# luisdamiano/sparseRGPs

Hardware: AMD Instinct MI355X
Metric: sparse-GP objective+gradient evals/sec at n=1e6, m=1024, d=8 (higher is better)
Workload: dtype f64; 1 GPU; C3: Titsias VI ELBO + gradient, n=1000000, m=1024, d=8, ard, P=10, knots fixed; n=1000000, m=1024, d=8, kernel=ard, parallelism=single

## Files before the change

include/sgp_diag.h:

```cpp
#ifndef SGP_DIAG_H
#define SGP_DIAG_H

#include <stdint.h>

#ifdef __cplusplus
extern "C" {
#endif

int sgp_diag_gj_pair(int device, int64_t m, const double* A, const double* B, double beta,
                     int per_step, double* invA, double* invS, double* logdet);

int sgp_diag_store_bw(int device, int64_t bytes, int reps, int pattern, double* gbs);

#ifdef __cplusplus
}
#endif
#endif
```

sparsergps_amd/_build.py:

```python
from __future__ import annotations

import os
import shutil
import subprocess

HERE = os.path.dirname(os.path.abspath(__file__))
ROOT = os.path.dirname(HERE)
CSRC = os.path.join(HERE, "csrc")
LIBDIR = os.path.join(HERE, "lib")
LIB = os.path.join(LIBDIR, "libsgp.so")
VARIANT_ROOT = os.path.join(ROOT, "tools", "ab")
SOURCES = ["capi.hip", "k_cov.hip", "k_mfma.hip", "k_dense.hip", "k_lap.hip", "multi.hip"]
HEADERS = ["sgp_internal.h", "sgp_probe.h", "sgp_multi.h", "sgp_pool.h",
           os.path.join("..", "..", "include", "sgp.h"),
           os.path.join("..", "..", "include", "sgp_diag.h")]
ARCH = "gfx950"


class HipccMissing(RuntimeError):
    """No hipcc on this machine (the only case in which an existing library may be reused)."""


def hipcc():
    for cand in (shutil.which("hipcc"), "/opt/rocm/bin/hipcc"):
        if cand and os.path.exists(cand):
            return cand
    raise HipccMissing("hipcc not found: cannot build libsgp.so")

# ... 114 lines not shown
        raise RuntimeError("SGP_HIPCC_DEFS is not honoured by the product build; "
                           "use sparsergps_amd._build.build_variant() for A/B libraries")
    return _build_into(LIBDIR, LIB, (), force, verbose)


def build_variant(name: str, defs=(), force: bool = False, verbose: bool = False,
                  rev: str | None = None) -> str:
    if not name or "/" in name or name.startswith("."):
        raise ValueError(f"bad variant name {name!r}")
    defs = ["-DSGP_PROBE_BUILD", *defs]
    outdir = os.path.join(VARIANT_ROOT, name)
    csrc = CSRC
    if rev is not None:
        src_root = os.path.join(outdir, "src")
        os.makedirs(src_root, exist_ok=True)
        for path in ["sparsergps_amd/csrc/" + f for f in SOURCES + HEADERS[:4]] + ["include/sgp.h", "include/sgp_diag.h"]:
            res = subprocess.run(["git", "-C", ROOT, "show", f"{rev}:{path}"],
                                 stdout=subprocess.PIPE, stderr=subprocess.PIPE)
            if res.returncode != 0:
                continue
            out = res.stdout
            dst = os.path.join(src_root, path)
            os.makedirs(os.path.dirname(dst), exist_ok=True)
            old = open(dst, "rb").read() if os.path.exists(dst) else None
            if old != out:
                with open(dst, "wb") as f:
                    f.write(out)
        csrc = os.path.join(src_root, "sparsergps_amd", "csrc")
    return _build_into(outdir, os.path.join(outdir, "libsgp.so"), defs, force, verbose, csrc)


# ... 9 lines not shown
```

sparsergps_amd/_lib.py:

```python
from __future__ import annotations

import ctypes as C
import os
import threading

from ._build import LIB, VARIANT_ROOT, HipccMissing, build

_lock = threading.Lock()
_lib = None

c_double_p = C.POINTER(C.c_double)
c_int_p = C.POINTER(C.c_int)

SGP_OK, SGP_EINVAL, SGP_ENOTPD, SGP_EHIP, SGP_ENOMEM = 0, 1, 2, 3, 4
KERNELS = {"sqexp": 0, "ard": 1, "exp": 2}
SGP_FLAG_R_DET = 1
SGP_FLAG_OBJ_ONLY = 2
SGP_PRED_VI, SGP_PRED_LAPLACE, SGP_PRED_FULL = 0, 1, 2
SGP_EXPO_ROWS = 0.0
FAMILIES = {"poisson": 0, "bernoulli": 1}

PROTOTYPES = {
    "sgp_last_error": (C.c_char_p, []),
    "sgp_abi_version": (C.c_int, []),
# ... 30 lines not shown
                                C.c_double, C.c_void_p]),
    "sgp_vi_phase2": (C.c_int, [C.c_void_p, C.c_void_p, C.c_int64, C.c_uint, C.c_void_p]),
    "sgp_vi_finish": (C.c_int, [C.c_void_p, C.c_void_p, c_double_p, c_double_p]),
    "sgp_fitc_red1_count": (C.c_int64, [C.c_int64]),
    "sgp_fitc_red2_count": (C.c_int64, [C.c_int, C.c_int, C.c_int64]),
    "sgp_fitc_phase1": (C.c_int, [C.c_void_p, C.c_int, c_double_p, c_double_p, C.c_int64, C.c_int64,
                                  C.c_double, C.c_void_p]),
    "sgp_fitc_phase2": (C.c_int, [C.c_void_p, C.c_void_p, C.c_int64, C.c_uint, C.c_void_p]),
    "sgp_fitc_finish": (C.c_int, [C.c_void_p, C.c_void_p, c_double_p, c_double_p]),
    "sgp_lap_set_f": (C.c_int, [C.c_void_p, c_double_p, C.c_double]),
    "sgp_lap_set_expo": (C.c_int, [C.c_void_p, c_double_p, C.c_double]),
    "sgp_lap_set_family": (C.c_int, [C.c_void_p, C.c_int]),
    "sgp_diag_gj_pair": (C.c_int, [C.c_int, C.c_int64, c_double_p, c_double_p, C.c_double, C.c_int,
                                   c_double_p, c_double_p, c_double_p]),
    "sgp_diag_store_bw": (C.c_int, [C.c_int, C.c_int64, C.c_int, C.c_int, c_double_p]),
    "sgp_lap_get_f": (C.c_int, [C.c_void_p, c_double_p]),
    "sgp_lap_get_grad_psi": (C.c_int, [C.c_void_p, c_double_p]),
    "sgp_lap_objective_values": (C.c_int, [C.c_void_p, c_double_p, C.c_int, c_int_p]),
    "sgp_eval_laplace": (C.c_int, [C.c_void_p, C.c_int, c_double_p, c_double_p, C.c_int64,
                                   C.c_int64, C.c_double, C.c_double, C.c_double, C.c_int,
                                   c_double_p, c_double_p, c_int_p]),
    "sgp_lap_red_count": (C.c_int64, [C.c_int, C.c_int, C.c_int64]),
    "sgp_lap_begin": (C.c_int, [C.c_void_p, C.c_int, c_double_p, c_double_p, C.c_int64, C.c_int64,
                                C.c_double, C.c_double, C.c_double, C.c_int, C.c_uint,
                                C.c_void_p, C.POINTER(C.c_int64)]),
    "sgp_lap_step": (C.c_int, [C.c_void_p, C.c_void_p, C.c_void_p, C.POINTER(C.c_int64), c_int_p,
                               c_double_p, c_double_p, c_int_p]),
    "sgp_lap_nr": (C.c_int, [C.c_void_p, C.c_int, c_double_p, c_double_p, C.c_int64, C.c_int64,
                             C.c_double, C.c_double, C.c_double, C.c_int, c_double_p, c_int_p]),
    "sgp_eval_full": (C.c_int, [C.c_void_p, C.c_int, c_double_p, C.c_double, C.c_uint,
# ... 94 lines not shown
```

sparsergps_amd/csrc/capi.hip:

```cpp
#include <math.h>

#include <cmath>
#include <stdarg.h>
#include <stdio.h>
#include <stdlib.h>
#include <string.h>
#include <time.h>

#include <algorithm>
#include <string>
#include <vector>

#include "../../include/sgp.h"
#include "../../include/sgp_diag.h"
#include "sgp_internal.h"

#ifdef SGP_HOST_PROBE
extern "C" __attribute__((visibility("default"))) double sgp_probe_t[4] = {0.0, 0.0, 0.0, 0.0};
#endif
#include "sgp_probe.h"
#include "sgp_multi.h"

namespace {

// ... 2887 lines not shown
                         dim3(256), 0, sg.s, buf.p, nrb, mp, (double)r);
    if (err == hipSuccess) err = hipGetLastError();
    if (err == hipSuccess) err = hipEventRecord(e1, sg.s);
    if (err == hipSuccess) err = hipEventSynchronize(e1);
    float ms = 0.0f;
    if (err == hipSuccess) err = hipEventElapsedTime(&ms, e0, e1);
    if (err == hipSuccess && r > 0 && ms > 0.0f) best = std::max(best, (double)used / (ms * 1e6));
  }
  (void)hipEventDestroy(e0);
  (void)hipEventDestroy(e1);
  HIPCHK(err);
  *gbs = best;
  return SGP_OK;
}

}
```

sparsergps_amd/csrc/k_mfma.hip:

```cpp
#include <algorithm>
#include <vector>

#include "sgp_internal.h"
#include "sgp_probe.h"

namespace {

constexpr int T128 = 128;
constexpr int BK = 16;
constexpr int SB = 144;
constexpr int SA = 17;
constexpr int SYRK_RGRP = 16;

__device__ __forceinline__ double wave_sum(double v) {
#pragma unroll
  for (int o = 32; o > 0; o >>= 1) v += __shfl_xor(v, o, 64);
  return v;
}

__device__ __forceinline__ int64_t xcd_remap(int64_t orig, int64_t nwg) {
  const int64_t x = orig % 8, q = nwg / 8, r = nwg % 8;
  const int64_t base = (x < r) ? x * (q + 1) : r * (q + 1) + (x - r) * q;
  return base + orig / 8;
}

__device__ __forceinline__ void load8(const double* __restrict__ g, double2 (&v)[4]) {
  const double2* p = reinterpret_cast<const double2*>(g);
#pragma unroll
  for (int q = 0; q < 4; ++q) v[q] = p[q];
}
__device__ __forceinline__ void store8(double* s, const double2 (&v)[4]) {
  double2* p = reinterpret_cast<double2*>(s);
#pragma unroll
  for (int q = 0; q < 4; ++q) p[q] = v[q];
}

__device__ __forceinline__ void syrk_group(int64_t gi, int nb, int wv, int& ta, int& tb, int& rs,
                                           int& cs, int& rp, int& cp) {
// ... 33 lines not shown
template <bool SPREAD = false, int PAT = 0, int NVMEM = 8, int NMFMA = 64>
__device__ __forceinline__ void mfma_interleave() {
#pragma unroll
  for (int i = 0; i < NMFMA; ++i) {
    __builtin_amdgcn_sched_group_barrier(0x008, 1, 0);
    if (i >= SGP_IL_VMEM0 && i < SGP_IL_VMEM0 + NVMEM)
      __builtin_amdgcn_sched_group_barrier(0x020, 1, 0);
    if (SPREAD ? (i & 1) == 0 : i < 32)
      __builtin_amdgcn_sched_group_barrier(0x100, 1, 0);
    constexpr int w0 = PAT == 2 ? NMFMA - 8 : PAT == 3 ? NMFMA / 2 : NMFMA - 16;
    if (PAT != 4 && i >= w0 && i < w0 + 8)
      __builtin_amdgcn_sched_group_barrier(0x200, 1, 0);
  }
}

template <int V, int WMODE, int TMODE>
__device__ __forceinline__ void syrk_dt_body(const double* __restrict__ K, int64_t mp,
                                             const double* __restrict__ w,
                                             const double* __restrict__ r,
                                             const double* __restrict__ tv, int t, int64_t rbeg,
                                             int nsteps, double (*Ka)[BK * SB], double (*ws)[BK],
                                             double (*rw)[BK], double& tacc, double& rrp,
                                             double* __restrict__ out) {
  constexpr int R0 = V, R1 = 7 - V, N0 = R0 + 1, N1 = R1 + 1;
  constexpr bool WITH_T = TMODE != 0;
  const int tid = threadIdx.x, lane = tid & 63;
  d4 acc0[N0], acc1[N1];
#pragma unroll
  for (int c = 0; c < N0; ++c) acc0[c] = d4{0.0, 0.0, 0.0, 0.0};
#pragma unroll
  for (int c = 0; c < N1; ++c) acc1[c] = d4{0.0, 0.0, 0.0, 0.0};
// ... 68 lines not shown
    SDT_SSTORE(cur ^ 1, more ? 1.0 : 0.0);
    if constexpr (SGP_SDT_IL && WMODE != 1) mfma_interleave<false, 2, 4, 36>();
    __syncthreads();
  }
#undef SDT_GLOAD
#undef SDT_SSTORE
  tacc = (t4[0] + t4[1]) + (t4[2] + t4[3]);
#pragma unroll
  for (int c = 0; c < N1; ++c)
#pragma unroll
    for (int hh = 0; hh < 2; ++hh) {
      if (hh == 0 && c >= N0) continue;
      const int R = hh == 0 ? R0 : R1;
      const d4& a = hh == 0 ? acc0[c] : acc1[c];
      const int rp = 2 * t + R / 4, cp = 2 * t + c / 4;
      double* blk = out + (int64_t)(rp * (rp + 1) / 2 + cp) * 4096;
#pragma unroll
      for (int q = 0; q < 4; ++q)
        blk[((R % 4) * 16 + (lane >> 4) + 4 * q) * 64 + (c % 4) * 16 + (lane & 15)] = a[q];
    }
}

template <int WMODE, int TMODE>
__device__ __forceinline__ void syrk_dtile(const double* __restrict__ K, int64_t n_pad,
                                           int64_t mp, const double* __restrict__ w,
                                           const double* __restrict__ r,
                                           const double* __restrict__ tv, int t, int nb,
                                           int64_t sd, int64_t chunk, double (*Ka)[BK * SB],
                                           double (*ws)[BK], double (*rw)[BK],
                                           double* __restrict__ out,
                                           double* __restrict__ slab_t,
// ... 207 lines not shown
  }
  if (!active) return;
  const int64_t bid = (int64_t)rp * (rp + 1) / 2 + cp;
  const int64_t nblk = (int64_t)(2 * nb) * (2 * nb + 1) / 2;
  double* out = slab + ((int64_t)split * nblk + bid) * 4096;
#pragma unroll
  for (int fm = 0; fm < 4; ++fm)
#pragma unroll
    for (int fn = 0; fn < 4; ++fn)
#pragma unroll
      for (int q = 0; q < 4; ++q) {
        const int row = fm * 16 + (lane >> 4) + 4 * q;
        const int col = fn * 16 + (lane & 15);
        out[row * 64 + col] = acc[fm][fn][q];
      }
}

__global__ void __launch_bounds__(256)
k_sqrt_rows(const double* __restrict__ w, int64_t n, double* __restrict__ sw) {
  const int64_t i = (int64_t)blockIdx.x * 256 + threadIdx.x;
  if (i < n) sw[i] = sqrt(w[i]);
}

__global__ void __launch_bounds__(256)
k_syrk_reduce_grp(double* __restrict__ slab, int splits, int64_t nblk) {
  const int64_t bid = blockIdx.y;
  const int e = blockIdx.x * 256 + threadIdx.x;
  const int s0 = blockIdx.z * SYRK_RGRP;
  const int s1 = s0 + SYRK_RGRP < splits ? s0 + SYRK_RGRP : splits;
  double a[SYRK_RGRP];
// ... 1170 lines not shown
  }
#pragma unroll
  for (int fm = 0; fm < 2; ++fm)
#pragma unroll
    for (int fn = 0; fn < 2; ++fn)
#pragma unroll
      for (int q = 0; q < 4; ++q) {
        const int64_t row = i0 + wr * 32 + fm * 16 + (lane >> 4) + 4 * q;
        const int64_t col = j0 + wc * 32 + fn * 16 + (lane & 15);
        double v = alpha * acc[fm][fn][q];
        if (beta != 0.0) v = fma(beta, C[row * ldc + col], v);
        C[row * ldc + col] = v;
      }
}

struct SyrkPlan {
  int nb, T, splits;
  int64_t chunk;
};

SyrkPlan syrk_plan(int64_t n_pad, int64_t mp) {
  constexpr int64_t kSlots = 512;
  SyrkPlan p;
  p.nb = (int)(mp / T128);
  p.T = p.nb * (p.nb + 1) / 2;
  const int64_t max_splits = n_pad / BK > 0 ? n_pad / BK : 1;
  int64_t best = 1;
  double best_fill = 0.0;
  for (int64_t rounds = 1; rounds <= 4; ++rounds) {
    int64_t sp = rounds * kSlots / p.T;
    if (sp < 1) sp = 1;
    if (sp > max_splits) sp = max_splits;
    const double fill = (double)(sp * p.T) / (double)(((sp * p.T + kSlots - 1) / kSlots) * kSlots);
    if (fill > best_fill + 1e-9) { best_fill = fill; best = sp; }
    if (best_fill >= 0.95) break;
  }
  int64_t chunk = (n_pad + best - 1) / best;
  chunk = (chunk + BK - 1) / BK * BK;
  p.chunk = chunk;
  p.splits = (int)((n_pad + chunk - 1) / chunk);
  return p;
}

static void syrk_group_panels(int64_t gi, int nb, int& ta, int& tb) {
  const int64_t noff = (int64_t)nb * (nb - 1) / 2;
  if (gi < noff) {
    int a = 1;
    while ((int64_t)(a + 1) * a / 2 <= gi) ++a;
    ta = a;
    tb = (int)(gi - (int64_t)a * (a - 1) / 2);
    return;
  }
  const int g = (int)(gi - noff), G = (3 * nb + 3) / 4, te = G + g / 3;
  ta = g;
  tb = te < nb ? te : g;
}

// ... 15 lines not shown
    bool ok = true;
    for (int p : order) {
      for (int sl = 0; sl < S && ok; ++sl) {
        bool placed = false;
        for (int gi : holders[p])
          if (used[gi] < 0) { used[gi] = p * S + sl; placed = true; break; }
        ok = placed;
      }
    }
    if (ok) {
      for (int gi = 0; gi < ngroups; ++gi) tmap[gi] = used[gi];
      return S;
    }
  }
  return 0;
}

SyrkPlan syrk_plan_blk(int64_t n_pad, int64_t mp) {
  SyrkPlan p = syrk_plan(n_pad, mp);
  const int nb = p.nb;
  const int groups = nb * (nb - 1) / 2 + (3 * nb + 3) / 4;
  constexpr int64_t kSlots = 512;
  const int64_t max_splits = n_pad / BK > 0 ? n_pad / BK : 1;
  int64_t best = 1;
  double best_fill = 0.0;
  for (int64_t rounds = 1; rounds <= 4; ++rounds) {
    int64_t sp = rounds * kSlots / groups;
    if (sp < 1) sp = 1;
    if (sp > max_splits) sp = max_splits;
    const double fill = (double)(sp * groups) /
                        (double)(((sp * groups + kSlots - 1) / kSlots) * kSlots);
    if (fill > best_fill + 1e-9) { best_fill = fill; best = sp; }
    if (best_fill >= 0.95) break;
  }
  int64_t chunk = (n_pad + best - 1) / best;
  chunk = (chunk + BK - 1) / BK * BK;
  p.T = groups;
  p.chunk = chunk;
  p.splits = (int)((n_pad + chunk - 1) / chunk);
  return p;
}

struct SyrkBal {
  bool on = false;
  int S_o = 0, S_d = 0;
  int64_t chunk_o = 0, chunk_d = 0;
};

static double syrk_dtile_cost(bool weighted, bool with_t) {
  return (double)SGP_SDT_W + (weighted ? (double)SGP_SDT_WW : 0.0) +
         (with_t ? (double)SGP_SDT_WT : 0.0);
}

static SyrkBal syrk_plan_bal(int64_t n_pad, int64_t mp, double wd, bool force) {
  SyrkBal b;
// ... 18 lines not shown
      best = T;
      b.chunk_o = co;
      b.chunk_d = cd;
      b.S_o = (int)((n_pad + co - 1) / co);
      b.S_d = (int)((n_pad + cd - 1) / cd);
    }
  }
  if (!b.on || force) return b;
  const SyrkPlan q = syrk_plan_blk(n_pad, mp);
  const int64_t rounds = ((int64_t)q.splits * q.T + kSlots - 1) / kSlots;
  const double T_pack = 64.0 * (double)q.chunk * (double)rounds;
  b.on = best < 0.98 * T_pack;
  return b;
}

static SyrkPlan syrk_plan_s256(int64_t n_pad) {
  SyrkPlan p;
  p.nb = 2;
  p.T = 2;
  constexpr int64_t kSlots = 512;
  const int64_t max_splits = n_pad / BK > 0 ? n_pad / BK : 1;
  int64_t sp = kSlots / p.T;
  if (sp > max_splits) sp = max_splits;
  int64_t chunk = (n_pad + sp - 1) / sp;
  chunk = (chunk + BK - 1) / BK * BK;
  p.chunk = chunk;
  p.splits = (int)((n_pad + chunk - 1) / chunk);
  return p;
}

// ... 2 lines not shown
bool syrk_use_s256(int64_t mp, bool with_t) { return mp == 256 && !with_t; }

namespace {

int64_t syrk_slab_doubles_mp(int64_t n_pad, int64_t mp) {
  SyrkPlan q = syrk_plan_blk(n_pad, mp);
  const int64_t nblk = (int64_t)(2 * q.nb) * (2 * q.nb + 1) / 2;
  int64_t need = (int64_t)q.splits * nblk * 4096 + (int64_t)q.splits * q.nb * T128 + q.splits +
                 n_pad;
  for (int v = 0; v < 3; ++v) {
    const SyrkBal bal = syrk_plan_bal(n_pad, mp, syrk_dtile_cost(v > 0, v > 1), v > 0);
    if (bal.on)
      need = std::max(need, (int64_t)(bal.S_o + bal.S_d) * nblk * 4096 +
                                (int64_t)std::max(bal.S_o, bal.S_d) * (q.nb * T128 + 1) + n_pad);
  }
  if (mp == 256) {
    SyrkPlan r = syrk_plan_s256(n_pad);
    need = std::max(need, (int64_t)r.splits * (10 * 4096 + 2 * T128 + 1) + n_pad);
  }
  return need;
}
}

int64_t syrk_slab_doubles(int64_t n_pad, int64_t mp) {
  int64_t need = 0;
  for (int64_t q = T128; q <= mp; q += T128) need = std::max(need, syrk_slab_doubles_mp(n_pad, q));
  return need;
}

hipError_t launch_syrk_aug(const double* K, int64_t n_pad, int64_t mp, const double* r,
                           const double* w, double* slab, int64_t slab_cap, double* red,
                           hipStream_t s, int part, const double* tv, int with_t,
                           const double* rr_src, bool packed, bool w_nonneg, unsigned* rsync) {
  if (packed && with_t) return hipErrorInvalidValue;
  {
    const bool s256 = syrk_use_s256(mp, with_t != 0);
    SyrkPlan q = s256 ? syrk_plan_s256(n_pad) : syrk_plan_blk(n_pad, mp);
    const bool wsq = w && w_nonneg && !with_t;
    bool use3 = !s256 && w && !wsq && SGP_SYRK_W3 && q.nb >= 3;
    SyrkBal bal;
    if (use3) bal = syrk_plan_bal(n_pad, mp, syrk_dtile_cost(true, with_t != 0), true);
    else if (!s256 && !with_t) bal = syrk_plan_bal(n_pad, mp, syrk_dtile_cost(false, false), false);
    if (use3 && !bal.on) use3 = false;
    if (bal.on) {
      q.T = q.nb * (q.nb - 1) / 2;
      q.splits = bal.S_o;
      q.chunk = bal.chunk_o;
    }
    const int64_t nblk = (int64_t)(2 * q.nb) * (2 * q.nb + 1) / 2;
    double* sl_s = slab;
    double* sl_d = sl_s + (int64_t)q.splits * nblk * 4096;
// ... 73 lines not shown
      if (bal.on && bal.S_d > SYRK_RGRP) {
        const unsigned ng = (unsigned)((bal.S_d + SYRK_RGRP - 1) / SYRK_RGRP);
        hipLaunchKernelGGL(k_syrk_reduce_grp, dim3(4096 / 256, (unsigned)nblk, ng), dim3(256), 0,
                           s, sl_d, bal.S_d, nblk);
        stride_d = SYRK_RGRP;
      }
      hipLaunchKernelGGL(k_syrk_reduce_blk, dim3(4096 / 256, (unsigned)nblk), dim3(256), 0, s,
                         sl_s, q.splits, nblk, mp, red, stride, rr_src,
                         red + (packed ? nblk * 4096 : mp * mp) + mp, packed ? 1 : 0,
                         bal.on ? sl_d : nullptr, bal.S_d, stride_d);
      if (with_t)
        hipLaunchKernelGGL(k_syrk_reduce_t, dim3((unsigned)((mp + 255) / 256)), dim3(256), 0, s,
                           sl_t, sl_rr, t_splits, q.nb, mp, red);
    }
    return hipGetLastError();
  }
}

int64_t syrk_packed_doubles(int64_t mp) {
  const int64_t nb64 = mp / 64;
  return nb64 * (nb64 + 1) / 2 * 4096;
}

hipError_t launch_unpack_lower64(const double* packed, int64_t mp, double* S, hipStream_t s) {
  hipLaunchKernelGGL(k_unpack_lower64, dim3((unsigned)((mp * mp + 255) / 256)), dim3(256), 0, s,
                     packed, mp, S);
  return hipGetLastError();
}

int64_t gemm_tn_splits(int64_t n_pad, int ntile) {
// ... 273 lines not shown
```

sparsergps_amd/csrc/sgp_internal.h:

```cpp
#pragma once
#include <hip/hip_runtime.h>
#include <stdint.h>

#define SGP_MAXD 32
#define SGP_TILE 128
#define SGP_DB 64
#define SGP_GJ_SYNC_WORDS (128 + 2 * 64 * 64)

typedef double d4 __attribute__((ext_vector_type(4)));

__device__ __forceinline__ double sgp_exp_nonpos(double x) {
  constexpr double c2 = 1.0 / 2, c3 = 1.0 / 6, c4 = 1.0 / 24, c5 = 1.0 / 120, c6 = 1.0 / 720,
                   c7 = 1.0 / 5040, c8 = 1.0 / 40320, c9 = 1.0 / 362880, c10 = 1.0 / 3628800,
                   c11 = 1.0 / 39916800, c12 = 1.0 / 479001600, c13 = 1.0 / 6227020800.0;
  const double k = __builtin_rint(x * 1.4426950408889634074);
  double r = __builtin_fma(-k, 6.93147180369123816490e-01, x);
  r = __builtin_fma(-k, 1.90821492927058770002e-10, r);
  double p = c13;
  p = __builtin_fma(p, r, c12);
  p = __builtin_fma(p, r, c11);
  p = __builtin_fma(p, r, c10);
  p = __builtin_fma(p, r, c9);
  p = __builtin_fma(p, r, c8);
  p = __builtin_fma(p, r, c7);
// ... 85 lines not shown
                               double* slab, int64_t slab_cap, int* nblocks, hipStream_t s);

hipError_t launch_syrk_aug(const double* K, int64_t n_pad, int64_t mp, const double* r,
                           const double* w, double* slab, int64_t slab_cap, double* red,
                           hipStream_t s, int part = 3,
                           const double* tv = nullptr,
                           int with_t = 1,
                           const double* rr_src = nullptr,
                           bool packed = false,
                           bool w_nonneg = false,
                           unsigned* rsync = nullptr);
#define SGP_SYRK_RSYNC_WORDS 4096
int64_t syrk_packed_doubles(int64_t mp);
hipError_t launch_unpack_lower64(const double* packed, int64_t mp, double* S, hipStream_t s);
int64_t syrk_slab_doubles(int64_t n_pad, int64_t mp);
bool syrk_use_s256(int64_t mp, bool with_t);
struct ConArgs {
  const double* r = nullptr;
  double invz = 0.0;
  const double* invz_vec = nullptr;
  const double* uvec = nullptr;
  const double* alpha_in = nullptr;
  const double* beta_in = nullptr;
  const double* vvec = nullptr;
  const double* rs_vec = nullptr;
  double rs = 1.0;
  const double* cdiag = nullptr;
  int count_a2 = 0;
  double* alpha_out = nullptr;
  bool vi_fold = false;
// ... 162 lines not shown
```

sparsergps_amd/csrc/sgp_probe.h:

```cpp
#pragma once

#if (defined(SGP_CON_TRACE) || defined(SGP_CON_NO_EPILOGUE) || defined(SGP_GJ_TRACE) ||       \
     defined(SGP_IL_VMEM0) || defined(SGP_CON_IL_PAT) || defined(SGP_SYRK_IL_PAT) ||          \
     defined(SGP_CON_IL_SPREAD) || defined(SGP_CON_SHMEM) ||                                  \
     defined(SGP_SYRK_BAL) || defined(SGP_SDT_IL) || defined(SGP_S256_IL) ||                  \
     defined(SGP_SDT_W) || defined(SGP_SDT_WW) || defined(SGP_SDT_WT) ||                      \
     defined(SGP_SYRK_W3) || defined(SGP_CON_ROWQ_KU) ||                                      \
     defined(SGP_LAP_RS_CFG) || defined(SGP_GJ_MM_UNROLL) || defined(SGP_VI_BUILD_NO_T) ||        \
     defined(SGP_GJ_STEPS) || defined(SGP_GJ_GMAX) || defined(SGP_CHAIN_US_STEP) ||         \
     defined(SGP_CHAIN_US_FIX) || defined(SGP_HOST_PROBE) || defined(SGP_BUILD_OCC_T2) ||      \
     defined(SGP_CON_EPI_PRIO) || defined(SGP_CON_PROBE_NO_EPI_MFMA) ||                       \
     defined(SGP_CON_PROBE_NO_KDMA)) &&      \
    !defined(SGP_PROBE_BUILD)
#error "timing probes and experiment knobs are for variant builds only (SGP_PROBE_BUILD)"
#endif

#ifndef SGP_CON_EPI_PRIO
#define SGP_CON_EPI_PRIO 0
#endif
#ifndef SGP_BUILD_OCC_T2
#define SGP_BUILD_OCC_T2 4
#endif
#ifndef SGP_IL_VMEM0
#define SGP_IL_VMEM0 0
#endif
#ifndef SGP_CON_IL_PAT
#define SGP_CON_IL_PAT 2
#endif
#ifndef SGP_SYRK_IL_PAT
#define SGP_SYRK_IL_PAT 0
#endif
#ifndef SGP_CON_IL_SPREAD
#define SGP_CON_IL_SPREAD false
#endif
#ifndef SGP_CON_SHMEM
#define SGP_CON_SHMEM 0
#endif
#ifndef SGP_SYRK_BAL
#define SGP_SYRK_BAL 1
#endif
#ifndef SGP_SDT_IL
#define SGP_SDT_IL 1
#endif
#ifndef SGP_SDT_W
#define SGP_SDT_W 38
#endif
#ifndef SGP_SDT_WW
#define SGP_SDT_WW 2
#endif
#ifndef SGP_SDT_WT
#define SGP_SDT_WT 6
#endif
#ifndef SGP_SYRK_W3
#define SGP_SYRK_W3 1
// ... 69 lines not shown
```

Measured before the change: 21.11 evals/s.

## Add load-balanced SYRK work plan mixing off-diagonal and diagonal segments

Adds a host-side planner that splits the K^T K SYRK into off-diagonal row bands and variable-length diagonal segments, so every workgroup gets a near-equal cost estimate. It also adds a new kernel that can run one off-diagonal segment plus one diagonal segment per workgroup, and a reduction kernel that sums the per-slab partials. The goal is to cut the tail imbalance of the earlier packed split plan in the unweighted SYRK path. The plan is cached per thread and is only used when its modelled makespan beats the packed plan. This brings more slab memory, extra reduction traffic and a more complex indexing scheme.

```diff
diff --git a/include/sgp_diag.h b/include/sgp_diag.h
--- a/include/sgp_diag.h
+++ b/include/sgp_diag.h
@@ -12,6 +12,9 @@
 
 int sgp_diag_store_bw(int device, int64_t bytes, int reps, int pattern, double* gbs);
 
+int sgp_diag_syrk_plan(int64_t n, int64_t m, int* plan, int* workgroups, double* t_balanced,
+                       double* t_packed);
+
 #ifdef __cplusplus
 }
 #endif
diff --git a/sparsergps_amd/_build.py b/sparsergps_amd/_build.py
--- a/sparsergps_amd/_build.py
+++ b/sparsergps_amd/_build.py
@@ -11,7 +11,8 @@
 LIB = os.path.join(LIBDIR, "libsgp.so")
 VARIANT_ROOT = os.path.join(ROOT, "tools", "ab")
 SOURCES = ["capi.hip", "k_cov.hip", "k_mfma.hip", "k_dense.hip", "k_lap.hip", "multi.hip"]
-HEADERS = ["sgp_internal.h", "sgp_probe.h", "sgp_multi.h", "sgp_pool.h",
+CSRC_HEADERS = ["sgp_internal.h", "sgp_probe.h", "sgp_multi.h", "sgp_pool.h", "sgp_syrk_plan.h"]
+HEADERS = [*CSRC_HEADERS,
            os.path.join("..", "..", "include", "sgp.h"),
            os.path.join("..", "..", "include", "sgp_diag.h")]
 ARCH = "gfx950"
@@ -156,7 +157,7 @@
     if rev is not None:
         src_root = os.path.join(outdir, "src")
         os.makedirs(src_root, exist_ok=True)
-        for path in ["sparsergps_amd/csrc/" + f for f in SOURCES + HEADERS[:4]] + ["include/sgp.h", "include/sgp_diag.h"]:
+        for path in ["sparsergps_amd/csrc/" + f for f in SOURCES + CSRC_HEADERS] + ["include/sgp.h", "include/sgp_diag.h"]:
             res = subprocess.run(["git", "-C", ROOT, "show", f"{rev}:{path}"],
                                  stdout=subprocess.PIPE, stderr=subprocess.PIPE)
             if res.returncode != 0:
diff --git a/sparsergps_amd/_lib.py b/sparsergps_amd/_lib.py
--- a/sparsergps_amd/_lib.py
+++ b/sparsergps_amd/_lib.py
@@ -68,6 +68,8 @@
     "sgp_diag_gj_pair": (C.c_int, [C.c_int, C.c_int64, c_double_p, c_double_p, C.c_double, C.c_int,
                                    c_double_p, c_double_p, c_double_p]),
     "sgp_diag_store_bw": (C.c_int, [C.c_int, C.c_int64, C.c_int, C.c_int, c_double_p]),
+    "sgp_diag_syrk_plan": (C.c_int, [C.c_int64, C.c_int64, c_int_p, c_int_p, c_double_p,
+                                     c_double_p]),
     "sgp_lap_get_f": (C.c_int, [C.c_void_p, c_double_p]),
     "sgp_lap_get_grad_psi": (C.c_int, [C.c_void_p, c_double_p]),
     "sgp_lap_objective_values": (C.c_int, [C.c_void_p, c_double_p, C.c_int, c_int_p]),
diff --git a/sparsergps_amd/csrc/capi.hip b/sparsergps_amd/csrc/capi.hip
--- a/sparsergps_amd/csrc/capi.hip
+++ b/sparsergps_amd/csrc/capi.hip
@@ -2925,4 +2925,15 @@
   return SGP_OK;
 }
 
-}
+int sgp_diag_syrk_plan(int64_t n, int64_t m, int* plan, int* workgroups, double* t_balanced,
+                       double* t_packed) {
+  if (n < 1 || m < 1 || !plan || !workgroups || !t_balanced || !t_packed) {
+    set_err("invalid sgp_diag_syrk_plan arguments");
+    return SGP_EINVAL;
+  }
+  syrk_plan_info(round_up(n, SGP_TILE), round_up(m, SGP_TILE), plan, workgroups, t_balanced,
+                 t_packed);
+  return SGP_OK;
+}
+
+}
diff --git a/sparsergps_amd/csrc/k_mfma.hip b/sparsergps_amd/csrc/k_mfma.hip
--- a/sparsergps_amd/csrc/k_mfma.hip
+++ b/sparsergps_amd/csrc/k_mfma.hip
@@ -3,6 +3,7 @@
 
 #include "sgp_internal.h"
 #include "sgp_probe.h"
+#include "sgp_syrk_plan.h"
 
 namespace {
 
@@ -19,9 +20,7 @@
 }
 
 __device__ __forceinline__ int64_t xcd_remap(int64_t orig, int64_t nwg) {
-  const int64_t x = orig % 8, q = nwg / 8, r = nwg % 8;
-  const int64_t base = (x < r) ? x * (q + 1) : r * (q + 1) + (x - r) * q;
-  return base + orig / 8;
+  return sgp_plan::xcd_remap(orig, nwg);
 }
 
 __device__ __forceinline__ void load8(const double* __restrict__ g, double2 (&v)[4]) {
@@ -85,7 +84,7 @@
   }
 }
 
-template <int V, int WMODE, int TMODE>
+template <int V, int WMODE, int TMODE, bool COMPACT = false>
 __device__ __forceinline__ void syrk_dt_body(const double* __restrict__ K, int64_t mp,
                                              const double* __restrict__ w,
                                              const double* __restrict__ r,
@@ -184,7 +183,8 @@
       const int R = hh == 0 ? R0 : R1;
       const d4& a = hh == 0 ? acc0[c] : acc1[c];
       const int rp = 2 * t + R / 4, cp = 2 * t + c / 4;
-      double* blk = out + (int64_t)(rp * (rp + 1) / 2 + cp) * 4096;
+      double* blk = out + (COMPACT ? (int64_t)(R / 4 + c / 4)
+                                   : (int64_t)(rp * (rp + 1) / 2 + cp)) * 4096;
 #pragma unroll
       for (int q = 0; q < 4; ++q)
         blk[((R % 4) * 16 + (lane >> 4) + 4 * q) * 64 + (c % 4) * 16 + (lane & 15)] = a[q];
@@ -422,6 +422,157 @@
         const int col = fn * 16 + (lane & 15);
         out[row * 64 + col] = acc[fm][fn][q];
       }
+}
+
+__device__ __forceinline__ void syrk_off_seg(const double* __restrict__ K, int64_t mp, int ta,
+                                             int tb, int64_t rbeg, int nsteps,
+                                             double (*Ka)[BK * SB], double (*Kb)[BK * SB],
+                                             double* __restrict__ out) {
+  const int tid = threadIdx.x, lane = tid & 63, wv = tid >> 6;
+  d4 acc[4][4];
+#pragma unroll
+  for (int a = 0; a < 4; ++a)
+#pragma unroll
+    for (int b = 0; b < 4; ++b) acc[a][b] = d4{0.0, 0.0, 0.0, 0.0};
+  const int lrow = tid >> 4, lc = tid & 15;
+  const double2* gA = reinterpret_cast<const double2*>(K + (rbeg + lrow) * mp + ta * (int64_t)T128) + lc;
+  const double2* gB = reinterpret_cast<const double2*>(K + (rbeg + lrow) * mp + tb * (int64_t)T128) + lc;
+  const int64_t gstep = BK * mp / 2;
+  double2 va0, va1, va2, va3, vb0, vb1, vb2, vb3;
+  const int ro = (wv >> 1) * 64, co = (wv & 1) * 64;
+#define SYRKO_GLOAD(step)                                                       \
+  {                                                                             \
+    const int64_t o_ = (int64_t)(step) * gstep;                                 \
+    va0 = gA[o_]; va1 = gA[o_ + 16]; va2 = gA[o_ + 32]; va3 = gA[o_ + 48];      \
+    vb0 = gB[o_]; vb1 = gB[o_ + 16]; vb2 = gB[o_ + 32]; vb3 = gB[o_ + 48];      \
+  }
+#define SYRKO_SSTORE(buf)                                                       \
+  {                                                                             \
+    double2* pa_ = reinterpret_cast<double2*>(&Ka[buf][lrow * SB]) + lc;        \
+    double2* pb_ = reinterpret_cast<double2*>(&Kb[buf][lrow * SB]) + lc;        \
+    pa_[0] = va0; pa_[16] = va1; pa_[32] = va2; pa_[48] = va3;                  \
+    pb_[0] = vb0; pb_[16] = vb1; pb_[32] = vb2; pb_[48] = vb3;                  \
+  }
+  SYRKO_GLOAD(0);
+  SYRKO_SSTORE(0);
+  __syncthreads();
+  for (int step = 0; step < nsteps; ++step) {
+    const int cur = step & 1;
+    const bool more = step + 1 < nsteps;
+    SYRKO_GLOAD(more ? step + 1 : step);
+    const double* As = Ka[cur] + ro;
+    const double* Bs = Kb[cur] + co;
+#pragma unroll
+    for (int kk = 0; kk < 4; ++kk) {
+      const int krow = kk * 4 + (lane >> 4);
+      double af[4], bf[4];
+#pragma unroll
+      for (int f = 0; f < 4; ++f) {
+        af[f] = As[krow * SB + f * 16 + (lane & 15)];
+        bf[f] = Bs[krow * SB + f * 16 + (lane & 15)];
+      }
+#pragma unroll
+      for (int fm = 0; fm < 4; ++fm)
+#pragma unroll
+        for (int fn = 0; fn < 4; ++fn)
+          acc[fm][fn] = __builtin_amdgcn_mfma_f64_16x16x4f64(af[fm], bf[fn], acc[fm][fn], 0, 0, 0);
+    }
+    SYRKO_SSTORE(cur ^ 1);
+    mfma_interleave<false, SGP_SYRK_IL_PAT, 8>();
+    __syncthreads();
+  }
+#undef SYRKO_GLOAD
+#undef SYRKO_SSTORE
+  double* blk = out + (int64_t)wv * 4096;
+#pragma unroll
+  for (int fm = 0; fm < 4; ++fm)
+#pragma unroll
+    for (int fn = 0; fn < 4; ++fn)
+#pragma unroll
+      for (int q = 0; q < 4; ++q) {
+        const int row = fm * 16 + (lane >> 4) + 4 * q;
+        const int col = fn * 16 + (lane & 15);
+        blk[row * 64 + col] = acc[fm][fn][q];
+      }
+}
+
+__device__ __forceinline__ void syrk_diag_seg(const double* __restrict__ K, int64_t mp, int t,
+                                              int64_t rbeg, int nsteps, double (*Ka)[BK * SB],
+                                              double* __restrict__ out) {
+  double tacc = 0.0, rrp = 0.0;
+  switch (threadIdx.x >> 6) {
+    case 0: syrk_dt_body<0, 0, 0, true>(K, mp, nullptr, nullptr, nullptr, t, rbeg, nsteps, Ka, nullptr, nullptr, tacc, rrp, out); break;
+    case 1: syrk_dt_body<1, 0, 0, true>(K, mp, nullptr, nullptr, nullptr, t, rbeg, nsteps, Ka, nullptr, nullptr, tacc, rrp, out); break;
+    case 2: syrk_dt_body<2, 0, 0, true>(K, mp, nullptr, nullptr, nullptr, t, rbeg, nsteps, Ka, nullptr, nullptr, tacc, rrp, out); break;
+    default: syrk_dt_body<3, 0, 0, true>(K, mp, nullptr, nullptr, nullptr, t, rbeg, nsteps, Ka, nullptr, nullptr, tacc, rrp, out); break;
+  }
+}
+
+__global__ void __launch_bounds__(256, 2)
+k_syrk_bal(const double* __restrict__ K, int64_t mp, sgp_plan::SyrkBalPlan p,
+           double* __restrict__ slab_o, double* __restrict__ slab_d) {
+  __shared__ __attribute__((aligned(16))) double Ka[2][BK * SB];
+  __shared__ __attribute__((aligned(16))) double Kb[2][BK * SB];
+  const int wg = (int)blockIdx.x < p.M ? (int)xcd_remap(blockIdx.x, p.M) : (int)blockIdx.x;
+  sgp_plan::SyrkSeg s0, s1;
+  sgp_plan::syrk_bp_segments(p, wg, s0, s1);
+  if (s0.kind == sgp_plan::SEG_OFF) {
+    int ta, tb;
+    sgp_plan::syrk_off_panels(s0.id, ta, tb);
+    syrk_off_seg(K, mp, ta, tb, s0.step0 * BK, s0.nsteps, Ka, Kb,
+                 slab_o + ((int64_t)s0.slab * p.noff + s0.id) * 4 * 4096);
+  } else if (s0.kind == sgp_plan::SEG_DIAG) {
+    syrk_diag_seg(K, mp, s0.id, s0.step0 * BK, s0.nsteps, Ka, slab_d + (int64_t)s0.slab * 3 * 4096);
+  }
+  if (s1.kind == sgp_plan::SEG_DIAG)
+    syrk_diag_seg(K, mp, s1.id, s1.step0 * BK, s1.nsteps, Ka, slab_d + (int64_t)s1.slab * 3 * 4096);
+}
+
+__global__ void __launch_bounds__(256)
+k_syrk_reduce_bal(const double* __restrict__ slab_o, const double* __restrict__ slab_d,
+                  sgp_plan::SyrkBalPlan p, int64_t mp, double* __restrict__ red,
+                  const double* __restrict__ rr_src, double* __restrict__ rr_dst, int packed) {
+  const int64_t bid = blockIdx.y;
+  const int e = blockIdx.x * 256 + threadIdx.x;
+  if (rr_src && bid == 0 && e < 8) rr_dst[e] = e == 0 ? *rr_src : 0.0;
+  int rp = (int)((sqrtf(8.0f * (float)bid + 1.0f) - 1.0f) * 0.5f);
+  while ((int64_t)(rp + 1) * (rp + 2) / 2 <= bid) ++rp;
+  while ((int64_t)rp * (rp + 1) / 2 > bid) --rp;
+  const int cp = (int)(bid - (int64_t)rp * (rp + 1) / 2);
+  const bool upper = rp == cp && (e / 64) / 16 < (e % 64) / 16;
+  if (upper && !packed) return;
+  if (!packed && rp == cp && (e / 64) < (e % 64)) return;
+  const double* src;
+  int64_t stride;
+  int cnt;
+  if (rp / 2 == cp / 2) {
+    const int t = rp / 2;
+    src = slab_d + ((int64_t)p.sfirst[t] * 3 + (rp & 1) + (cp & 1)) * 4096 + e;
+    stride = 3 * 4096;
+    cnt = p.sfirst[t + 1] - p.sfirst[t];
+  } else {
+    const int a = rp / 2, b = cp / 2, gi = a * (a - 1) / 2 + b;
+    src = slab_o + ((int64_t)gi * 4 + (rp & 1) * 2 + (cp & 1)) * 4096 + e;
+    stride = (int64_t)p.noff * 4 * 4096;
+    cnt = p.B;
+  }
+  double v = 0.0;
+  if (!upper)
+    for (int s0 = 0; s0 < cnt; s0 += 16) {
+      double a[16];
+#pragma unroll
+      for (int q = 0; q < 16; ++q) a[q] = s0 + q < cnt ? src[(int64_t)(s0 + q) * stride] : 0.0;
+#pragma unroll
+      for (int q = 0; q < 16; ++q)
+        if (s0 + q < cnt) v += a[q];
+    }
+  if (packed) {
+    red[bid * 4096 + e] = v;
+    return;
+  }
+  const int64_t a = (int64_t)rp * 64 + e / 64, b = (int64_t)cp * 64 + e % 64;
+  red[a * mp + b] = v;
+  red[b * mp + a] = v;
 }
 
 __global__ void __launch_bounds__(256)
@@ -1622,33 +1773,9 @@
       }
 }
 
-struct SyrkPlan {
-  int nb, T, splits;
-  int64_t chunk;
-};
-
-SyrkPlan syrk_plan(int64_t n_pad, int64_t mp) {
-  constexpr int64_t kSlots = 512;
-  SyrkPlan p;
-  p.nb = (int)(mp / T128);
-  p.T = p.nb * (p.nb + 1) / 2;
-  const int64_t max_splits = n_pad / BK > 0 ? n_pad / BK : 1;
-  int64_t best = 1;
-  double best_fill = 0.0;
-  for (int64_t rounds = 1; rounds <= 4; ++rounds) {
-    int64_t sp = rounds * kSlots / p.T;
-    if (sp < 1) sp = 1;
-    if (sp > max_splits) sp = max_splits;
-    const double fill = (double)(sp * p.T) / (double)(((sp * p.T + kSlots - 1) / kSlots) * kSlots);
-    if (fill > best_fill + 1e-9) { best_fill = fill; best = sp; }
-    if (best_fill >= 0.95) break;
-  }
-  int64_t chunk = (n_pad + best - 1) / best;
-  chunk = (chunk + BK - 1) / BK * BK;
-  p.chunk = chunk;
-  p.splits = (int)((n_pad + chunk - 1) / chunk);
-  return p;
-}
+using sgp_plan::SyrkPlan;
+using sgp_plan::syrk_plan;
+using sgp_plan::syrk_plan_blk;
 
 static void syrk_group_panels(int64_t gi, int nb, int& ta, int& tb) {
   const int64_t noff = (int64_t)nb * (nb - 1) / 2;
@@ -1694,31 +1821,6 @@
     }
   }
   return 0;
-}
-
-SyrkPlan syrk_plan_blk(int64_t n_pad, int64_t mp) {
-  SyrkPlan p = syrk_plan(n_pad, mp);
-  const int nb = p.nb;
-  const int groups = nb * (nb - 1) / 2 + (3 * nb + 3) / 4;
-  constexpr int64_t kSlots = 512;
-  const int64_t max_splits = n_pad / BK > 0 ? n_pad / BK : 1;
-  int64_t best = 1;
-  double best_fill = 0.0;
-  for (int64_t rounds = 1; rounds <= 4; ++rounds) {
-    int64_t sp = rounds * kSlots / groups;
-    if (sp < 1) sp = 1;
-    if (sp > max_splits) sp = max_splits;
-    const double fill = (double)(sp * groups) /
-                        (double)(((sp * groups + kSlots - 1) / kSlots) * kSlots);
-    if (fill > best_fill + 1e-9) { best_fill = fill; best = sp; }
-    if (best_fill >= 0.95) break;
-  }
-  int64_t chunk = (n_pad + best - 1) / best;
-  chunk = (chunk + BK - 1) / BK * BK;
-  p.T = groups;
-  p.chunk = chunk;
-  p.splits = (int)((n_pad + chunk - 1) / chunk);
-  return p;
 }
 
 struct SyrkBal {
@@ -1767,6 +1869,18 @@
   return b;
 }
 
+static sgp_plan::SyrkBalPlan syrk_plan_wb(int64_t n_pad, int64_t mp) {
+  if (!SGP_SYRK_WB) return sgp_plan::SyrkBalPlan{};
+  thread_local int64_t last_n = -1, last_mp = -1;
+  thread_local sgp_plan::SyrkBalPlan last{};
+  if (last_n != n_pad || last_mp != mp) {
+    last = sgp_plan::syrk_plan_balanced(n_pad, mp, SGP_SYRK_WB_SLOTS, (double)SGP_SDT_W);
+    last_n = n_pad;
+    last_mp = mp;
+  }
+  return last;
+}
+
 static SyrkPlan syrk_plan_s256(int64_t n_pad) {
   SyrkPlan p;
   p.nb = 2;
@@ -1799,6 +1913,8 @@
       need = std::max(need, (int64_t)(bal.S_o + bal.S_d) * nblk * 4096 +
                                 (int64_t)std::max(bal.S_o, bal.S_d) * (q.nb * T128 + 1) + n_pad);
   }
+  const sgp_plan::SyrkBalPlan wb = syrk_plan_wb(n_pad, mp);
+  if (wb.on) need = std::max(need, sgp_plan::syrk_bp_slab_doubles(wb));
   if (mp == 256) {
     SyrkPlan r = syrk_plan_s256(n_pad);
     need = std::max(need, (int64_t)r.splits * (10 * 4096 + 2 * T128 + 1) + n_pad);
@@ -1820,6 +1936,24 @@
   if (packed && with_t) return hipErrorInvalidValue;
   {
     const bool s256 = syrk_use_s256(mp, with_t != 0);
+    if (!s256 && !with_t && !w) {
+      const sgp_plan::SyrkBalPlan wb = syrk_plan_wb(n_pad, mp);
+      if (wb.on) {
+        if (sgp_plan::syrk_bp_slab_doubles(wb) > slab_cap) return hipErrorInvalidValue;
+        double* sl_o = slab;
+        double* sl_d = slab + sgp_plan::syrk_bp_off_doubles(wb);
+        if (part & 1)
+          hipLaunchKernelGGL(k_syrk_bal, dim3((unsigned)wb.nwg), dim3(256), 0, s, K, mp, wb, sl_o,
+                             sl_d);
+        if (part & 2) {
+          const int64_t nblk = (int64_t)(2 * wb.nb) * (2 * wb.nb + 1) / 2;
+          hipLaunchKernelGGL(k_syrk_reduce_bal, dim3(4096 / 256, (unsigned)nblk), dim3(256), 0, s,
+                             sl_o, sl_d, wb, mp, red, rr_src,
+                             red + (packed ? nblk * 4096 : mp * mp) + mp, packed ? 1 : 0);
+        }
+        return hipGetLastError();
+      }
+    }
     SyrkPlan q = s256 ? syrk_plan_s256(n_pad) : syrk_plan_blk(n_pad, mp);
     const bool wsq = w && w_nonneg && !with_t;
     bool use3 = !s256 && w && !wsq && SGP_SYRK_W3 && q.nb >= 3;
@@ -1923,6 +2057,25 @@
                            sl_t, sl_rr, t_splits, q.nb, mp, red);
     }
     return hipGetLastError();
+  }
+}
+
+void syrk_plan_info(int64_t n_pad, int64_t mp, int* plan, int* nwg, double* t_bal,
+                    double* t_pack) {
+  const sgp_plan::SyrkBalPlan wb = syrk_plan_wb(n_pad, mp);
+  *t_bal = wb.T_bal;
+  *t_pack = wb.T_pack;
+  if (syrk_use_s256(mp, false)) {
+    *plan = 3;
+    *nwg = syrk_plan_s256(n_pad).splits * 2;
+  } else if (wb.on) {
+    *plan = 2;
+    *nwg = wb.nwg;
+  } else {
+    const SyrkBal bal = syrk_plan_bal(n_pad, mp, syrk_dtile_cost(false, false), false);
+    const SyrkPlan q = syrk_plan_blk(n_pad, mp);
+    *plan = bal.on ? 1 : 0;
+    *nwg = bal.on ? bal.S_o * (q.nb * (q.nb - 1) / 2) + bal.S_d * q.nb : q.splits * q.T;
   }
 }
 
diff --git a/sparsergps_amd/csrc/sgp_internal.h b/sparsergps_amd/csrc/sgp_internal.h
--- a/sparsergps_amd/csrc/sgp_internal.h
+++ b/sparsergps_amd/csrc/sgp_internal.h
@@ -123,6 +123,7 @@
 int64_t syrk_packed_doubles(int64_t mp);
 hipError_t launch_unpack_lower64(const double* packed, int64_t mp, double* S, hipStream_t s);
 int64_t syrk_slab_doubles(int64_t n_pad, int64_t mp);
+void syrk_plan_info(int64_t n_pad, int64_t mp, int* plan, int* nwg, double* t_bal, double* t_pack);
 bool syrk_use_s256(int64_t mp, bool with_t);
 struct ConArgs {
   const double* r = nullptr;
diff --git a/sparsergps_amd/csrc/sgp_probe.h b/sparsergps_amd/csrc/sgp_probe.h
--- a/sparsergps_amd/csrc/sgp_probe.h
+++ b/sparsergps_amd/csrc/sgp_probe.h
@@ -3,7 +3,8 @@
 #if (defined(SGP_CON_TRACE) || defined(SGP_CON_NO_EPILOGUE) || defined(SGP_GJ_TRACE) ||       \
      defined(SGP_IL_VMEM0) || defined(SGP_CON_IL_PAT) || defined(SGP_SYRK_IL_PAT) ||          \
      defined(SGP_CON_IL_SPREAD) || defined(SGP_CON_SHMEM) ||                                  \
-     defined(SGP_SYRK_BAL) || defined(SGP_SDT_IL) || defined(SGP_S256_IL) ||                  \
+     defined(SGP_SYRK_BAL) || defined(SGP_SYRK_WB) || defined(SGP_SYRK_WB_SLOTS) ||           \
+     defined(SGP_SDT_IL) || defined(SGP_S256_IL) ||                  \
      defined(SGP_SDT_W) || defined(SGP_SDT_WW) || defined(SGP_SDT_WT) ||                      \
      defined(SGP_SYRK_W3) || defined(SGP_CON_ROWQ_KU) ||                                      \
      defined(SGP_LAP_RS_CFG) || defined(SGP_GJ_MM_UNROLL) || defined(SGP_VI_BUILD_NO_T) ||        \
@@ -38,6 +39,12 @@
 #endif
 #ifndef SGP_SYRK_BAL
 #define SGP_SYRK_BAL 1
+#endif
+#ifndef SGP_SYRK_WB
+#define SGP_SYRK_WB 1
+#endif
+#ifndef SGP_SYRK_WB_SLOTS
+#define SGP_SYRK_WB_SLOTS 512
 #endif
 #ifndef SGP_SDT_IL
 #define SGP_SDT_IL 1
diff --git a/sparsergps_amd/csrc/sgp_syrk_plan.h b/sparsergps_amd/csrc/sgp_syrk_plan.h
--- /dev/null
+++ b/sparsergps_amd/csrc/sgp_syrk_plan.h
@@ -0,0 +1,324 @@
+#pragma once
+
+#include <stdint.h>
+
+#if defined(__HIPCC__)
+#define SGP_HD __host__ __device__ inline
+#else
+#define SGP_HD inline
+#endif
+
+namespace sgp_plan {
+
+constexpr int kStep = 16;
+constexpr int kTile = 128;
+constexpr int kMaxNb = 31;
+
+SGP_HD int64_t xcd_remap(int64_t orig, int64_t nwg) {
+  const int64_t x = orig % 8, q = nwg / 8, r = nwg % 8;
+  const int64_t base = (x < r) ? x * (q + 1) : r * (q + 1) + (x - r) * q;
+  return base + orig / 8;
+}
+
+struct SyrkPlan {
+  int nb, T, splits;
+  int64_t chunk;
+};
+
+inline SyrkPlan syrk_plan(int64_t n_pad, int64_t mp, int64_t kSlots = 512) {
+  SyrkPlan p;
+  p.nb = (int)(mp / kTile);
+  p.T = p.nb * (p.nb + 1) / 2;
+  const int64_t max_splits = n_pad / kStep > 0 ? n_pad / kStep : 1;
+  int64_t best = 1;
+  double best_fill = 0.0;
+  for (int64_t rounds = 1; rounds <= 4; ++rounds) {
+    int64_t sp = rounds * kSlots / p.T;
+    if (sp < 1) sp = 1;
+    if (sp > max_splits) sp = max_splits;
+    const double fill = (double)(sp * p.T) / (double)(((sp * p.T + kSlots - 1) / kSlots) * kSlots);
+    if (fill > best_fill + 1e-9) { best_fill = fill; best = sp; }
+    if (best_fill >= 0.95) break;
+  }
+  int64_t chunk = (n_pad + best - 1) / best;
+  chunk = (chunk + kStep - 1) / kStep * kStep;
+  p.chunk = chunk;
+  p.splits = (int)((n_pad + chunk - 1) / chunk);
+  return p;
+}
+
+inline SyrkPlan syrk_plan_blk(int64_t n_pad, int64_t mp, int64_t kSlots = 512) {
+  SyrkPlan p = syrk_plan(n_pad, mp, kSlots);
+  const int nb = p.nb;
+  const int groups = nb * (nb - 1) / 2 + (3 * nb + 3) / 4;
+  const int64_t max_splits = n_pad / kStep > 0 ? n_pad / kStep : 1;
+  int64_t best = 1;
+  double best_fill = 0.0;
+  for (int64_t rounds = 1; rounds <= 4; ++rounds) {
+    int64_t sp = rounds * kSlots / groups;
+    if (sp < 1) sp = 1;
+    if (sp > max_splits) sp = max_splits;
+    const double fill = (double)(sp * groups) /
+                        (double)(((sp * groups + kSlots - 1) / kSlots) * kSlots);
+    if (fill > best_fill + 1e-9) { best_fill = fill; best = sp; }
+    if (best_fill >= 0.95) break;
+  }
+  int64_t chunk = (n_pad + best - 1) / best;
+  chunk = (chunk + kStep - 1) / kStep * kStep;
+  p.T = groups;
+  p.chunk = chunk;
+  p.splits = (int)((n_pad + chunk - 1) / chunk);
+  return p;
+}
+
+inline double syrk_packed_makespan(int64_t n_pad, int64_t mp, int64_t kSlots, double c0) {
+  const SyrkPlan q = syrk_plan_blk(n_pad, mp, kSlots);
+  const int64_t rounds = ((int64_t)q.splits * q.T + kSlots - 1) / kSlots;
+  return (64.0 * (double)(q.chunk / kStep) + c0) * (double)rounds;
+}
+
+SGP_HD void syrk_off_panels(int gi, int& a, int& b) {
+  int x = 1;
+  while ((x + 1) * x / 2 <= gi) ++x;
+  a = x;
+  b = gi - x * (x - 1) / 2;
+}
+
+enum { SEG_NONE = 0, SEG_OFF = 1, SEG_DIAG = 2 };
+
+struct SyrkSeg {
+  int kind;
+  int id;
+  int64_t step0;
+  int nsteps;
+  int slab;
+};
+
+struct SyrkBalPlan {
+  int on;
+  int nb, noff;
+  int B;
+  int M;
+  int nwg;
+  int Ld;
+  int e;
+  int xfirst;
+  int64_t N;
+  int64_t afirst[kMaxNb + 1];
+  int dseg[kMaxNb];
+  int pfirst[kMaxNb + 1];
+  int sfirst[kMaxNb + 1];
+  double T_bal, T_pack;
+};
+
+SGP_HD int64_t syrk_bp_band(const SyrkBalPlan& p, int s) {
+  const int64_t q = p.N / p.B, r = p.N % p.B;
+  return s * q + (s < r ? s : r);
+}
+
+SGP_HD void syrk_bp_segments(const SyrkBalPlan& p, int wg, SyrkSeg& s0, SyrkSeg& s1) {
+  s0 = s1 = SyrkSeg{SEG_NONE, 0, 0, 0, 0};
+  if (wg < p.M) {
+    const int band = wg / p.noff;
+    s0.kind = SEG_OFF;
+    s0.id = wg % p.noff;
+    s0.step0 = syrk_bp_band(p, band);
+    s0.nsteps = (int)(syrk_bp_band(p, band + 1) - s0.step0);
+    s0.slab = band;
+    if (wg >= p.pfirst[p.nb]) return;
+    int t = 0;
+    while (wg >= p.pfirst[t + 1]) ++t;
+    const int i = wg - p.pfirst[t];
+    s1.kind = SEG_DIAG;
+    s1.id = t;
+    const int x0 = p.pfirst[t] > p.xfirst ? p.pfirst[t] : p.xfirst;
+    s1.step0 = (p.afirst[t + 1] - p.afirst[t]) + (int64_t)i * p.e + (wg > x0 ? wg - x0 : 0);
+    s1.nsteps = p.e + (wg >= p.xfirst ? 1 : 0);
+    s1.slab = p.sfirst[t] + p.dseg[t] + i;
+    return;
+  }
+  const int j = wg - p.M;
+  const int64_t A = p.afirst[p.nb], x0 = (int64_t)j * p.Ld;
+  const int64_t x1 = x0 + p.Ld < A ? x0 + p.Ld : A;
+  int t = 0;
+  while (x0 >= p.afirst[t + 1]) ++t;
+  const int64_t end0 = x1 < p.afirst[t + 1] ? x1 : p.afirst[t + 1];
+  s0.kind = SEG_DIAG;
+  s0.id = t;
+  s0.step0 = x0 - p.afirst[t];
+  s0.nsteps = (int)(end0 - x0);
+  s0.slab = p.sfirst[t] + (j - (int)(p.afirst[t] / p.Ld));
+  if (x1 > end0) {
+    s1.kind = SEG_DIAG;
+    s1.id = t + 1;
+    s1.step0 = 0;
+    s1.nsteps = (int)(x1 - end0);
+    s1.slab = p.sfirst[t + 1];
+  }
+}
+
+SGP_HD double syrk_bp_cost(const SyrkSeg& s, double wd, double c0) {
+  if (s.kind == SEG_NONE) return 0.0;
+  return (s.kind == SEG_OFF ? 64.0 : wd) * (double)s.nsteps + c0;
+}
+
+inline int64_t syrk_bp_off_doubles(const SyrkBalPlan& p) {
+  return (int64_t)p.B * p.noff * 4 * 4096;
+}
+inline int64_t syrk_bp_slab_doubles(const SyrkBalPlan& p) {
+  return syrk_bp_off_doubles(p) + (int64_t)p.sfirst[p.nb] * 3 * 4096;
+}
+
+namespace detail {
+struct Deal {
+  bool ok;
+  int Ld, e;
+  int64_t A;
+  double T;
+};
+inline int syrk_bp_xfirst(int64_t N, int nb, int B, double wd) {
+  const int noff = nb * (nb - 1) / 2;
+  return N % B == 0 || wd > 64.0 ? B * noff : (int)(N % B) * noff;
+}
+inline int64_t syrk_bp_pieces(int nb, int M, int xfirst, int e, int t, int64_t* steps) {
+  *steps = 0;
+  if (e <= 0) return 0;
+  const int64_t q = M / nb, r = M % nb, k = q + (t < r ? 1 : 0);
+  const int64_t first = t * q + (t < r ? t : r), x0 = first > xfirst ? first : xfirst;
+  *steps = k * e + (first + k > x0 ? first + k - x0 : 0);
+  return k;
+}
+inline Deal syrk_bp_deal(int64_t N, int nb, int B, int D, double wd, double c0, int e) {
+  const int M = B * (nb * (nb - 1) / 2);
+  Deal d{false, 0, e, 0, 0.0};
+  const int xfirst = syrk_bp_xfirst(N, nb, B, wd);
+  int64_t K = 0, amin = N;
+  d.A = 0;
+  for (int t = 0; t < nb; ++t) {
+    int64_t st;
+    K += syrk_bp_pieces(nb, M, xfirst, e, t, &st);
+    if (N - st < amin) amin = N - st;
+    d.A += N - st;
+  }
+  if (amin < 1) return d;
+  const int64_t Ld = (d.A + D - 1) / D;
+  d.Ld = (int)Ld;
+  const double f = 64.0 * (double)((N + B - 1) / B) + c0 + (K > 0 ? wd * (double)e + c0 : 0.0);
+  const double g = wd * (double)Ld + 2.0 * c0;
+  d.T = f > g ? f : g;
+  d.ok = Ld >= 1 && Ld <= amin && (e == 0 || K > 0);
+  int64_t fill = (int64_t)((d.T - 2.0 * c0) / wd);
+  if (fill > amin) fill = amin;
+  if (d.ok && fill > Ld) d.Ld = (int)fill;
+  return d;
+}
+inline Deal syrk_bp_best(int64_t N, int nb, int B, int D, double wd, double c0) {
+  Deal best = syrk_bp_deal(N, nb, B, D, wd, c0, 0);
+  int64_t lo = 1, hi = N / 2;
+  while (lo < hi) {
+    const int64_t mid = lo + (hi - lo) / 2;
+    const Deal d = syrk_bp_deal(N, nb, B, D, wd, c0, (int)mid);
+    const double g = wd * (double)((d.A + D - 1) / D) + 2.0 * c0;
+    if (d.T > g || !d.ok) hi = mid;
+    else lo = mid + 1;
+  }
+  for (int64_t e = lo > 2 ? lo - 2 : 1; e <= lo + 1 && e <= N / 2; ++e) {
+    const Deal d = syrk_bp_deal(N, nb, B, D, wd, c0, (int)e);
+    if (d.ok && (!best.ok || d.T < best.T)) best = d;
+  }
+  return best;
+}
+}
+
+inline SyrkBalPlan syrk_bp_build(int64_t N, int nb, int B, const detail::Deal& d, double wd) {
+  SyrkBalPlan p{};
+  p.nb = nb;
+  p.noff = nb * (nb - 1) / 2;
+  p.B = B;
+  p.M = B * p.noff;
+  p.N = N;
+  p.Ld = d.Ld;
+  p.e = d.e;
+  p.xfirst = detail::syrk_bp_xfirst(N, nb, B, wd);
+  p.T_bal = d.T;
+  p.afirst[0] = 0;
+  p.pfirst[0] = 0;
+  p.sfirst[0] = 0;
+  for (int t = 0; t < nb; ++t) {
+    int64_t st;
+    const int64_t k = detail::syrk_bp_pieces(nb, p.M, p.xfirst, p.e, t, &st), a = N - st;
+    p.afirst[t + 1] = p.afirst[t] + a;
+    p.dseg[t] = a > 0 ? (int)((p.afirst[t + 1] - 1) / p.Ld - p.afirst[t] / p.Ld + 1) : 0;
+    p.pfirst[t + 1] = p.pfirst[t] + (int)k;
+    p.sfirst[t + 1] = p.sfirst[t] + p.dseg[t] + (int)k;
+  }
+  p.nwg = p.M + (int)((p.afirst[nb] + p.Ld - 1) / p.Ld);
+  return p;
+}
+
+inline void syrk_bp_spread(const SyrkBalPlan& p, double wd, double c0, double* mx, double* mean) {
+  double sum = 0.0;
+  *mx = 0.0;
+  for (int wg = 0; wg < p.nwg; ++wg) {
+    SyrkSeg s0, s1;
+    syrk_bp_segments(p, wg, s0, s1);
+    const double c = syrk_bp_cost(s0, wd, c0) + syrk_bp_cost(s1, wd, c0);
+    sum += c;
+    if (c > *mx) *mx = c;
+  }
+  *mean = p.nwg > 0 ? sum / (double)p.nwg : 0.0;
+}
+inline bool syrk_bp_balanced(const SyrkBalPlan& p, double wd, double c0) {
+  double mx, mean;
+  syrk_bp_spread(p, wd, c0, &mx, &mean);
+  return mx <= mean + 64.0;
+}
+
+inline SyrkBalPlan syrk_plan_balanced(int64_t n_pad, int64_t mp, int slots, double wd,
+                                      double c0 = 8.0) {
+  SyrkBalPlan none{};
+  none.T_pack = mp >= kTile && n_pad >= kStep ? syrk_packed_makespan(n_pad, mp, 512, c0) : 0.0;
+  const int nb = (int)(mp / kTile);
+  const int64_t N = n_pad / kStep;
+  if (nb < 3 || nb > kMaxNb || N < 1 || wd <= 0.0 || c0 < 0.0) return none;
+  const int noff = nb * (nb - 1) / 2;
+  int Bmax = (slots - nb) / noff;
+  if ((int64_t)Bmax > N) Bmax = (int)N;
+  if (slots < nb || Bmax < 1) return none;
+  double Tmin = 0.0;
+  for (int b = 1; b <= Bmax; ++b) {
+    const detail::Deal d = detail::syrk_bp_best(N, nb, b, slots - b * noff, wd, c0);
+    if (d.ok && (Tmin == 0.0 || d.T < Tmin)) Tmin = d.T;
+  }
+  if (Tmin == 0.0) return none;
+  SyrkBalPlan bal[512 / 3 + 1];
+  double Tbb = 0.0;
+  for (int b = 1; b <= Bmax && b <= 512 / 3; ++b) {
+    bal[b].nwg = 0;
+    const detail::Deal d0 = detail::syrk_bp_best(N, nb, b, slots - b * noff, wd, c0);
+    if (!d0.ok || d0.T > 1.005 * Tmin) continue;
+    for (int64_t e = d0.e > 2 ? d0.e - 2 : 0; e <= N / 2; ++e) {
+      const detail::Deal d = detail::syrk_bp_deal(N, nb, b, slots - b * noff, wd, c0, (int)e);
+      if (e > d0.e && (!d.ok || d.T > 1.005 * Tmin)) break;
+      if (!d.ok || d.T > 1.005 * Tmin || (bal[b].nwg > 0 && d.T >= bal[b].T_bal)) continue;
+      const SyrkBalPlan q = syrk_bp_build(N, nb, b, d, wd);
+      if (syrk_bp_balanced(q, wd, c0)) bal[b] = q;
+    }
+    if (bal[b].nwg > 0 && (Tbb == 0.0 || bal[b].T_bal < Tbb)) Tbb = bal[b].T_bal;
+  }
+  SyrkBalPlan p{};
+  for (int b = 1; b <= Bmax && b <= 512 / 3 && p.nwg == 0; ++b) {
+    if (Tbb > 0.0) {
+      if (bal[b].nwg > 0 && bal[b].T_bal <= 1.001 * Tbb) p = bal[b];
+    } else {
+      const detail::Deal d = detail::syrk_bp_best(N, nb, b, slots - b * noff, wd, c0);
+      if (d.ok && d.T <= 1.001 * Tmin) p = syrk_bp_build(N, nb, b, d, wd);
+    }
+  }
+  if (p.nwg == 0) return none;
+  p.T_pack = none.T_pack;
+  p.on = p.T_bal < 0.98 * p.T_pack ? 1 : 0;
+  return p;
+}
+
+}
```

Result: faster. 21.38 evals/s (median of 6 runs) (+1.3%).
